# asalimil/Nonlinear-MPC-for-collision-free-and-deadlock-free-navigation-of-multiple-nonholonomic-mobile-robots

Hardware: AMD Instinct MI355X
Metric: NMPC solves/sec (batched swarms), N_robots=6, N=20 (higher is better)
Workload: dtype f64

## Files before the change

nonlinear-mpc-for-collision-free-and-deadlock-free-navigation-of-multiple-nonholonomic-mobile-robots_amd/csrc/nmpc_solve_col.hip:

```cpp
#include "nmpc_solve_common.h"

namespace nmpc {

__device__ __forceinline__ double lane_read(double v, int lane)
{
    return __hiloint2double(__builtin_amdgcn_readlane(__double2hiint(v), lane), __builtin_amdgcn_readlane(__double2loint(v), lane));
}
#ifndef NMPC_COL_GB
#define NMPC_COL_GB ((M_ == 6) ? (NX + 2) / 2 : NX + 1)
#endif
#ifndef NMPC_FW_PD
#define NMPC_FW_PD ((M_ <= 6) ? 2 : 1)
#endif
#ifndef NMPC_FW_FAKE
#define NMPC_FW_FAKE 0
#endif
#ifndef NMPC_COL_DPP
#define NMPC_COL_DPP 1
#endif
#ifndef NMPC_COL_WAVES_SMALL
#define NMPC_COL_WAVES_SMALL 1
#endif
#ifndef NMPC_COL_WAVES_MID
#define NMPC_COL_WAVES_MID 1
// ... 208 lines not shown
            for (int e = tid; e < N * NU; e += TPB) wo[(size_t)N1 * NX + e] = U[e];
            if (P.lam_g) for (int e = tid; e < P.ng; e += TPB) P.lam_g[inst * (size_t)P.ng + e] = 0.0;
            if (P.lam_x) for (int e = tid; e < P.nvar; e += TPB) P.lam_x[inst * (size_t)P.nvar + e] = 0.0;
            if (P.lam_p) for (int e = tid; e < 2 * NX; e += TPB) P.lam_p[inst * (size_t)(2 * NX) + e] = 0.0;
            if (tid == 0) {
                if (obj_out) obj_out[inst] = NAN;
                if (status_out) status_out[inst] = NMPC_STATUS_INFEASIBLE_X0;
                if (iters_out) iters_out[inst] = 0;
                if (kkt_out) kkt_out[inst] = INFINITY;
            }
            return;
        }
    }

    auto pair_ij = [&](int q, int &i, int &j) { pair_of<M_>(q, i, j); };

    auto trig = [&]() {
        for (int it = tid; it < N * M_; it += TPB) {
            int k = it / M_, i = it - k * M_;
            double s, c;
            sincos(X[k * NX + 3 * i + 2], &s, &c);
            SN[it] = s; CS[it] = c;
        }
    };
    auto merit_t = [&](auto elc, double a, double &fv, double &lg, double &th, double &ec_, double &eh_) {
        constexpr bool EL = decltype(elc)::value;
        double fs = 0.0, t = 0.0, mc = 0.0, mh = 0.0;
        LogSum ls;
        double pr = 1.0;
        auto brow = [&](double sv, double h0, double jd, double ht) {
            double st = sv + a * (jd + (h0 - sv));
            pr *= st;
            double r = fabs(ht - st);
            t += r; mh = fmax(mh, r);
        };
        for (int it = tid; it < N * M_; it += TPB) {
            int k = it / M_, i = it - k * M_;
            const int ox = k * NX + 3 * i, ou = k * NU + 2 * i;
            double x0 = X[ox] + a * DX[ox], x1 = X[ox + 1] + a * DX[ox + 1], x2 = X[ox + 2] + a * DX[ox + 2];
            double n0 = X[ox + NX] + a * DX[ox + NX], n1 = X[ox + NX + 1] + a * DX[ox + NX + 1], n2 = X[ox + NX + 2] + a * DX[ox + NX + 2];
            double u0 = U[ou] + a * DU[ou], u1 = U[ou + 1] + a * DU[ou + 1];
            double s, c;
            if (a == 0.0) { s = SN[it]; c = CS[it]; } else sincos(x2, &s, &c);
            double c0 = fabs(defect_xy(n0, x0, T * u0, c)), c1 = fabs(defect_xy(n1, x1, T * u0, s)), c2 = fabs(defect_th(n2, x2, T, u1));
            t += c0 + c1 + c2; mc = fmax(mc, fmax(c0, fmax(c1, c2)));
            double e0 = x0 - XS[3 * i], e1 = x1 - XS[3 * i + 1], e2 = x2 - XS[3 * i + 2];
            fs += P.q[0] * e0 * e0 + P.q[1] * e1 * e1 + P.q[2] * e2 * e2 + P.r[0] * u0 * u0 + P.r[1] * u1 * u1;
            brow(SUL[ou], U[ou] + P.vmax, DU[ou], u0 + P.vmax); brow(SUU[ou], P.vmax - U[ou], -DU[ou], P.vmax - u0);
            brow(SUL[ou + 1], U[ou + 1] + P.wmax, DU[ou + 1], u1 + P.wmax); brow(SUU[ou + 1], P.wmax - U[ou + 1], -DU[ou + 1], P.wmax - u1);
            pr *= ((n0 + P.xymax) * (P.xymax - n0)) * ((n1 + P.xymax) * (P.xymax - n1));
            if (THB) pr *= (n2 + P.thmax) * (P.thmax - n2);
            ls.add(pr);
            pr = 1.0;
        }
        for (int it = tid; it < (N - 1) * NPA; it += TPB) {
            int k = 1 + it / NPd, q = it - (k - 1) * NP, i, j;
            pair_ij(q, i, j);
            const int oi = k * NX + 3 * i, oj = k * NX + 3 * j;
            double dx = (X[oi] + a * DX[oi]) - (X[oj] + a * DX[oj]), dy = (X[oi + 1] + a * DX[oi + 1]) - (X[oj + 1] + a * DX[oj + 1]);
            double h = h_pair(dx, dy, P.dmin2);
            double sv = SPp[k * NP + q], tv = 0.0;
            if constexpr (EL) {
                tv = TPp[k * NP + q];
                if (a != 0.0) {
                    double ex = X[oi] - X[oj], ey = X[oi + 1] - X[oj + 1], ds, dz, dt;
                    el_step(mu, rho, sv, ZPp[k * NP + q], tv, h_pair(ex, ey, P.dmin2), jd_pair(ex, ey, DX[oi] - DX[oj], DX[oi + 1] - DX[oj + 1]), ds, dz, dt);
                    sv += a * ds; tv += a * dt;
                }
                ls.add(tv); fs += rho * tv;
            } else if (a != 0.0) {
                double ex = X[oi] - X[oj], ey = X[oi + 1] - X[oj + 1];
                sv += a * ds_pair(ex, ey, DX[oi] - DX[oj], DX[oi + 1] - DX[oj + 1], P.dmin2, sv);
            }
            ls.add(sv);
            double r = fabs(h - sv + tv);
            t += r; mh = fmax(mh, r);
        }
        for (int it = tid; it < (N - 1) * MK; it += TPB) {
            int k = 1 + it / MK, e = it - (k - 1) * MK, i = e / K, o = e - i * K;
            const int oi = k * NX + 3 * i;
            double px = X[oi] + a * DX[oi], py = X[oi + 1] + a * DX[oi + 1];
            double h = h_obs(r_obs(px - OB(k, o, 0), py - OB(k, o, 1)), P.robdim, OB(k, o, 2), P.margin);
            double sv = SO[k * MK + e], tv = 0.0;
            if constexpr (EL) {
                tv = TOb[k * MK + e];
                if (a != 0.0) {
                    double ex = X[oi] - OB(k, o, 0), ey = X[oi + 1] - OB(k, o, 1), rr = r_obs(ex, ey), ds, dz, dt;
                    el_step(mu, rho, sv, ZO[k * MK + e], tv, h_obs(rr, P.robdim, OB(k, o, 2), P.margin), jd_obs(ex, ey, rr, DX[oi], DX[oi + 1]), ds, dz, dt);
                    sv += a * ds; tv += a * dt;
                }
                ls.add(tv); fs += rho * tv;
            } else if (a != 0.0) {
                double ex = X[oi] - OB(k, o, 0), ey = X[oi + 1] - OB(k, o, 1), rr = r_obs(ex, ey);
// ... 3 lines not shown
            double r = fabs(h - sv + tv);
            t += r; mh = fmax(mh, r);
        }
        fv = wsum<TPB>(fs, RED); lg = wlogsum<TPB>(ls, RED); th = wsum<TPB>(t, RED);
        ec_ = wmax<TPB>(mc, RED); eh_ = wmax<TPB>(mh, RED);
    };
    auto merit = [&](double a, double &fv, double &lg, double &th, double &ec_, double &eh_) {
        if (el) merit_t(std::true_type{}, a, fv, lg, th, ec_, eh_); else merit_t(std::false_type{}, a, fv, lg, th, ec_, eh_);
    };

    for (int it = tid; it < N * M_; it += TPB) {
        int k = it / M_, i = it - k * M_;
        if (i == 0) { gpack[(size_t)k * G::PACK + G::PK_T] = T; gpack[(size_t)k * G::PACK + G::PK_ZERO] = 0.0; }
    }
    for (int q = tid; q < 3 * NP; q += TPB) gpack[G::PK_E + q] = 0.0;
    if (!prs)
        for (int e = tid; e < (N - 1) * 3 * NP; e += TPB) gpack[(size_t)(1 + e / (3 * NPd)) * G::PACK + G::PK_E + e % (3 * NPd)] = 0.0;
    auto init_barrier = [&]() {
        for (int it = tid; it < N1 * NP; it += TPB) {
            int k = it / NPd, q = it - k * NP;
            if (k >= 1 && k <= N - 1 && prs) {
                int i, j; pair_ij(q, i, j);
                double dx = X[k * NX + 3 * i] - X[k * NX + 3 * j], dy = X[k * NX + 3 * i + 1] - X[k * NX + 3 * j + 1];
                const double hv = h_pair(dx, dy, P.dmin2);
                if (el) {
                    const double tv = fmax(bp, bp - hv), sv = hv + tv;
                    TPp[it] = tv; SPp[it] = sv; ZPp[it] = fmin(mu / sv, 0.5 * rho);
                } else {
                double sv = fmax(hv, bp);
                SPp[it] = sv; ZPp[it] = mu / sv;
// ... 62 lines not shown
        }
        __syncthreads();
    }
    trig();
    __syncthreads();
    init_barrier();
    merit(0.0, f, lgs, th0, e_c, e_h);
    delta_last = 0.0; nu_pen = 1.0; need_shift = false; mcount = 0; restarting = false;
    PROF_T(0);

    for (;;) {
        double e_d = 0.0, lsum = 0.0, zsum = 0.0, szmax = 0.0, szmin = INFINITY;
#ifdef NMPC_PROFILE
        double dbg_code = -1.0, dbg_v[4] = {0, 0, 0, 0};
#endif
        for (int it = tid; it < N * M_; it += TPB) {
            int k = it / M_, i = it - k * M_, kk = k + 1;
            const double *x = X + kk * NX;
            double r0 = LAM[kk * NX + 3 * i], r1 = LAM[kk * NX + 3 * i + 1], r2 = LAM[kk * NX + 3 * i + 2];
            lsum += fabs(r0) + fabs(r1) + fabs(r2);
            if (kk < N) {
                const double *ln = LAM + (kk + 1) * NX + 3 * i;
                double v = U[kk * NU + 2 * i];
                double a = -T * v * SN[kk * M_ + i], b = T * v * CS[kk * M_ + i];
                r0 += 2 * P.q[0] * (x[3 * i] - XS[3 * i]) - ln[0];
                r1 += 2 * P.q[1] * (x[3 * i + 1] - XS[3 * i + 1]) - ln[1];
                r2 += 2 * P.q[2] * (x[3 * i + 2] - XS[3 * i + 2]) - (ln[2] + a * ln[0] + b * ln[1]);
            }
            double j0, j1, j2 = 0.0;
            {
                const int sb = kk * NXB + (2 + THB) * i;
                double zl0 = ZXL[sb], zu0 = ZXU[sb], zl1 = ZXL[sb + 1], zu1 = ZXU[sb + 1];
                j0 = zl0 - zu0; j1 = zl1 - zu1;
                zsum += zl0 + zu0 + zl1 + zu1;
                double p0 = (x[3 * i] + P.xymax) * zl0, p1 = (P.xymax - x[3 * i]) * zu0, p2 = (x[3 * i + 1] + P.xymax) * zl1, p3 = (P.xymax - x[3 * i + 1]) * zu1;
                szmax = fmax(szmax, fmax(fmax(p0, p1), fmax(p2, p3))); szmin = fmin(szmin, fmin(fmin(p0, p1), fmin(p2, p3)));
                if (THB) {
                    double zl2 = ZXL[sb + 2], zu2 = ZXU[sb + 2];
                    j2 = zl2 - zu2; zsum += zl2 + zu2;
                    double p4 = (x[3 * i + 2] + P.thmax) * zl2, p5 = (P.thmax - x[3 * i + 2]) * zu2;
                    szmax = fmax(szmax, fmax(p4, p5)); szmin = fmin(szmin, fmin(p4, p5));
                }
            }
            if (kk <= N - 1) {
                const double xi = x[3 * i], yi = x[3 * i + 1];
                if (prs) {
                    double zq[MPN];
                    static_for<0, M_ - 1>([&](auto pc) { constexpr int p = decltype(pc)::value; zq[p] = ZPp[kk * NP + pidx_any<M_>(i, p + (p >= i ? 1 : 0))]; });
                    static_for<0, M_ - 1>([&](auto pc) {
                        constexpr int p = decltype(pc)::value;
                        const int j = p + (p >= i ? 1 : 0);
                        j0 += 2 * (xi - x[3 * j]) * zq[p]; j1 += 2 * (yi - x[3 * j + 1]) * zq[p];
                    });
                }
                for (int o = 0; o < K; o++) {
                    double dx = xi - OB(kk, o, 0), dy = yi - OB(kk, o, 1), rr = r_obs(dx, dy), z = ZO[kk * MK + i * K + o];
                    j0 += qdiv(dx, rr) * z; j1 += qdiv(dy, rr) * z;
                }
            }
#ifdef NMPC_PROFILE
            { double m3 = fmax(fabs(r0 - j0), fmax(fabs(r1 - j1), fabs(r2 - j2)));
              if (m3 > e_d) { dbg_code = 1000.0 * kk + 10.0 * i + (fabs(r0 - j0) == m3 ? 0 : (fabs(r1 - j1) == m3 ? 1 : 2)); dbg_v[0] = r0 - j0; dbg_v[1] = r1 - j1; dbg_v[2] = r2 - j2; dbg_v[3] = r2; } }
#endif
            e_d = fmax(e_d, fmax(fabs(r0 - j0), fmax(fabs(r1 - j1), fabs(r2 - j2))));
            const double *ln = LAM + (k + 1) * NX + 3 * i, *u = U + k * NU + 2 * i;
            double c = CS[it], s = SN[it];
            double zl0 = ZUL[k * NU + 2 * i], zu0 = ZUU[k * NU + 2 * i], zl1 = ZUL[k * NU + 2 * i + 1], zu1 = ZUU[k * NU + 2 * i + 1];
            double rv = 2 * P.r[0] * u[0] - T * (c * ln[0] + s * ln[1]) - (zl0 - zu0);
            double rw = 2 * P.r[1] * u[1] - T * ln[2] - (zl1 - zu1);
#ifdef NMPC_PROFILE
            if (fmax(fabs(rv), fabs(rw)) > e_d) { dbg_code = 1000.0 * k + 10.0 * i + (fabs(rv) > fabs(rw) ? 5 : 6); dbg_v[0] = rv; dbg_v[1] = rw; dbg_v[2] = zl0 - zu0; dbg_v[3] = zl1 - zu1; }
#endif
            e_d = fmax(e_d, fmax(fabs(rv), fabs(rw)));
            zsum += zl0 + zu0 + zl1 + zu1;
            double p0 = SUL[k * NU + 2 * i] * zl0, p1 = SUU[k * NU + 2 * i] * zu0, p2 = SUL[k * NU + 2 * i + 1] * zl1, p3 = SUU[k * NU + 2 * i + 1] * zu1;
            szmax = fmax(szmax, fmax(fmax(p0, p1), fmax(p2, p3))); szmin = fmin(szmin, fmin(fmin(p0, p1), fmin(p2, p3)));
        }
        for (int it = tid; it < (N - 1) * NPA; it += TPB) {
            double zv = ZPp[NP + it], pz = SPp[NP + it] * zv;
            zsum += zv; szmax = fmax(szmax, pz); szmin = fmin(szmin, pz);
        }
        for (int it = tid; it < (N - 1) * MK; it += TPB) {
            double zv = ZO[MK + it], pz = SO[MK + it] * zv;
            zsum += zv; szmax = fmax(szmax, pz); szmin = fmin(szmin, pz);
        }
        if (el) {
            for (int it = tid; it < (N - 1) * NPA; it += TPB) { const double pt = TPp[NP + it] * (rho - ZPp[NP + it]); szmax = fmax(szmax, pt); szmin = fmin(szmin, pt); }
            for (int it = tid; it < (N - 1) * MK; it += TPB) { const double pt = TOb[MK + it] * (rho - ZO[MK + it]); szmax = fmax(szmax, pt); szmin = fmin(szmin, pt); }
        }
#ifdef NMPC_PROFILE
        { double my = e_d; double gm = wmax<TPB>(e_d, RED);
          if (prof_out && (int)inst == P.trace_inst && iter < 2040 && my == gm) {
              double *tr = reinterpret_cast<double *>(prof_out + 12 + 16 * 2048) + (size_t)iter * 8;
              tr[0] = dbg_code; tr[1] = dbg_v[0]; tr[2] = dbg_v[1]; tr[3] = dbg_v[2]; tr[4] = dbg_v[3]; } }
#endif
        e_d = wmax<TPB>(e_d, RED); lsum = wsum<TPB>(lsum, RED); zsum = wsum<TPB>(zsum, RED);
        szmax = wmax<TPB>(szmax, RED); szmin = wmin<TPB>(szmin, RED);
        const double smax = 100.0;
        double s_d = fmax(smax, (lsum + zsum) / ((double)(N * NX) + n_ineq)) / smax;
        double s_c = fmax(smax, zsum / fmax(n_ineq, 1.0)) / smax;
        double E0 = fmax(fmax(e_d / s_d, e_c), fmax(e_h, szmax / s_c));
        kkt = E0;
        auto cold_retry = [&]() { cold = true; n_cold++; it_base = iter; restarting = true; el = n_cold >= 2; mu = P.mu_init; n_tiny = 0; n_restart = 0; };
        if (!(E0 == E0)) { if (n_cold < NMPC_COLD_RETRIES && iter < P.max_iter) cold_retry(); else status = NMPC_STATUS_NUMERIC; break; }
        if (E0 <= P.tol) {
            status = NMPC_STATUS_CONVERGED;
            if (el) {
                double tmax = 0.0;
                for (int it = tid; it < (N - 1) * NPA; it += TPB) tmax = fmax(tmax, TPp[NP + it]);
                for (int it = tid; it < (N - 1) * MK; it += TPB) tmax = fmax(tmax, TOb[MK + it]);
                if (wmax<TPB>(tmax, RED) > NMPC_X0_TOL) status = NMPC_STATUS_STALLED;
            }
            break;
        }
        if (iter >= P.max_iter) { status = NMPC_STATUS_MAX_ITER; break; }
        if (n_cold < NMPC_COLD_RETRIES && iter - it_base >= NMPC_COLD_RETRY_ITERS) { cold_retry(); break; }
        const double mu_min = P.tol / 10.0;
        for (;;) {
            double cm = fmax(fabs(szmax - mu), fabs(szmin - mu));
            double Emu = fmax(fmax(e_d / s_d, e_c), fmax(e_h, cm / s_c));
            if (mu > mu_min && Emu <= 10.0 * mu) mu = fmax(mu_min, fmin(0.2 * mu, pow(mu, 1.5)));
            else break;
        }
        const double tau = fmax(0.99, 1.0 - mu);
        PROF_T(1);

        auto stage_packs = [&](auto elc) {
        constexpr bool EL = decltype(elc)::value;
        for (int it = tid; it < N1 * M_; it += TPB) {
            int k = it / M_, i = it - k * M_;
            const double *x = X + k * NX;
            double *pk = gpack + (size_t)k * G::PACK;
            double g0 = 0.0, g1 = 0.0, g2 = 0.0, h0 = 0.0, h1 = 0.0, h2 = 0.0, hxy = 0.0;
            if (k >= 1) {
                if (k < N) {
                    g0 = 2 * P.q[0] * (x[3 * i] - XS[3 * i]); g1 = 2 * P.q[1] * (x[3 * i + 1] - XS[3 * i + 1]); g2 = 2 * P.q[2] * (x[3 * i + 2] - XS[3 * i + 2]);
                    h0 = 2 * P.q[0]; h1 = 2 * P.q[1]; h2 = 2 * P.q[2];
                }
                const int sb = k * NXB + (2 + THB) * i;
                {
                    auto bv = [&](double sv, double zv, double hv, double &hd) { double sg = qdiv(zv, sv); hd += sg; return qdiv(mu, sv) - sg * (hv - sv); };
                    g0 -= bv(x[3 * i] + P.xymax, ZXL[sb], x[3 * i] + P.xymax, h0) - bv(P.xymax - x[3 * i], ZXU[sb], P.xymax - x[3 * i], h0);
                    g1 -= bv(x[3 * i + 1] + P.xymax, ZXL[sb + 1], x[3 * i + 1] + P.xymax, h1) - bv(P.xymax - x[3 * i + 1], ZXU[sb + 1], P.xymax - x[3 * i + 1], h1);
                    if (THB) g2 -= bv(x[3 * i + 2] + P.thmax, ZXL[sb + 2], x[3 * i + 2] + P.thmax, h2) - bv(P.thmax - x[3 * i + 2], ZXU[sb + 2], P.thmax - x[3 * i + 2], h2);
// ... 44 lines not shown
                }
                {
                    double *cf = pk + G::PK_CF + 4 * i;
                    cf[0] = T * c; cf[1] = T * s; cf[2] = -T * u[0] * s; cf[3] = T * u[0] * c;
                }
                const double *xn = x + NX;
                pk[G::PK_C + 3 * i] = defect_xy(xn[3 * i], x[3 * i], T * u[0], c);
                pk[G::PK_C + 3 * i + 1] = defect_xy(xn[3 * i + 1], x[3 * i + 1], T * u[0], s);
                pk[G::PK_C + 3 * i + 2] = defect_th(xn[3 * i + 2], x[3 * i + 2], T, u[1]);
                pk[G::PK_HVT + i] = hvt;
            }
            pk[G::PK_G + NU + 3 * i] = g0; pk[G::PK_G + NU + 3 * i + 1] = g1; pk[G::PK_G + NU + 3 * i + 2] = g2;
            pk[G::PK_HD + NU + 3 * i] = h0; pk[G::PK_HD + NU + 3 * i + 1] = h1; pk[G::PK_HD + NU + 3 * i + 2] = h2;
            pk[G::PK_HXY + i] = hxy;
        }
        for (int it = tid; it < (N - 1) * NPA; it += TPB) {
            int k = 1 + it / NPd, q = it - (k - 1) * NP, i, j;
            pair_ij(q, i, j);
            double dx = X[k * NX + 3 * i] - X[k * NX + 3 * j], dy = X[k * NX + 3 * i + 1] - X[k * NX + 3 * j + 1];
            double zz = ZPp[k * NP + q], sg;
            if constexpr (EL) { double v_; el_sigma(mu, rho, SPp[k * NP + q], zz, TPp[k * NP + q], h_pair(dx, dy, P.dmin2), sg, v_); }
            else sg = qdiv(zz, SPp[k * NP + q]);
            double *pk = gpack + (size_t)k * G::PACK + G::PK_E + 3 * q;
            pk[0] = -(4 * sg * dx * dx - 2 * zz); pk[1] = -(4 * sg * dx * dy); pk[2] = -(4 * sg * dy * dy - 2 * zz);
        }
        };
        if (el) stage_packs(std::true_type{}); else stage_packs(std::false_type{});
        __syncthreads();
        PROF_T(2);

        double delta = need_shift ? fmax(1e-20, 0.25 * delta_last) : 0.0;
        int ntry = 0;
        bool ok;
        int kst = N - 1;
        for (;;) {
            ok = true;
            int kf = 0;
            if (TPBK == 64 || tid < 64) {
            constexpr int TPB = 64;
            if constexpr (RP) {
            const int rh = tid >> 5, rw = (tid >> 4) & 1, rn = tid & 15;
            const bool cc_ = rn < NC;
// ... 477 lines not shown
#if NMPC_FUSE_DPHI
            dphi_b += qdiv(ds, sv);
#endif
            return zv + dz;
        };
        auto fbe = [&](double sv, double zv, double tv, double hv, double jd) -> double {
            double ds, dz, dt;
            el_step(mu, rho, sv, zv, tv, hv, jd, ds, dz, dt);
            if (ds < 0.0) a_p = fmin(a_p, qdiv(-tau * sv, ds));
            if (dt < 0.0) a_p = fmin(a_p, qdiv(-tau * tv, dt));
            if (dz < 0.0) a_d = fmin(a_d, qdiv(-tau * zv, dz));
            if (dz > 0.0) a_d = fmin(a_d, qdiv(tau * (rho - zv), dz));
            dphi_b += qdiv(ds, sv) + qdiv(dt, tv) - qdiv(rho, mu) * dt;
            return zv + dz;
        };
        for (int e = tid; e < N * NU; e += TPB) {
            int c = e % NU;
            double lo = lbu(c), u = U[e], du = DU[e], sl = SUL[e], su = SUU[e];
            fb(sl, ZUL[e], du + ((u - lo) - sl)); fb(su, ZUU[e], -du + ((-lo - u) - su));
        }
        for (int e = tid; e < N * NXB; e += TPB) {
            int k = 1 + e / NXB, s = e - (k - 1) * NXB;
            double v = X[k * NX + bst(s)], dv = DX[k * NX + bst(s)], b = bvl(s), sl = v + b, su = b - v;
            fb(sl, ZXL[k * NXB + s], dv + ((v + b) - sl)); fb(su, ZXU[k * NXB + s], -dv + ((b - v) - su));
        }
        if (!el) {
        for (int it = tid; it < (N - 1) * NPA; it += TPB) {
            int k = 1 + it / NPd, q = it - (k - 1) * NP, i, j;
            pair_ij(q, i, j);
            const int oi = k * NX + 3 * i, oj = k * NX + 3 * j;
            double ex = X[oi] - X[oj], ey = X[oi + 1] - X[oj + 1], sv = SPp[k * NP + q];
            double ds = ds_pair(ex, ey, DX[oi] - DX[oj], DX[oi + 1] - DX[oj + 1], P.dmin2, sv);
            mult_max = fmax(mult_max, fabs(fb(sv, ZPp[k * NP + q], ds)));
        }
        for (int it = tid; it < (N - 1) * MK; it += TPB) {
            int k = 1 + it / MK, e = it - (k - 1) * MK, i = e / K, o = e - i * K;
            const int oi = k * NX + 3 * i;
            double ex = X[oi] - OB(k, o, 0), ey = X[oi + 1] - OB(k, o, 1), rr = r_obs(ex, ey), sv = SO[k * MK + e];
            double ds = ds_obs(ex, ey, rr, DX[oi], DX[oi + 1], h_obs(rr, P.robdim, OB(k, o, 2), P.margin), sv);
            mult_max = fmax(mult_max, fabs(fb(sv, ZO[k * MK + e], ds)));
        }
        } else {
        for (int it = tid; it < (N - 1) * NPA; it += TPB) {
            int k = 1 + it / NPd, q = it - (k - 1) * NP, i, j;
            pair_ij(q, i, j);
            const int oi = k * NX + 3 * i, oj = k * NX + 3 * j;
            double ex = X[oi] - X[oj], ey = X[oi + 1] - X[oj + 1];
            mult_max = fmax(mult_max, fabs(fbe(SPp[k * NP + q], ZPp[k * NP + q], TPp[k * NP + q], h_pair(ex, ey, P.dmin2), jd_pair(ex, ey, DX[oi] - DX[oj], DX[oi + 1] - DX[oj + 1]))));
        }
        for (int it = tid; it < (N - 1) * MK; it += TPB) {
            int k = 1 + it / MK, e = it - (k - 1) * MK, i = e / K, o = e - i * K;
            const int oi = k * NX + 3 * i;
            double ex = X[oi] - OB(k, o, 0), ey = X[oi + 1] - OB(k, o, 1), rr = r_obs(ex, ey);
            mult_max = fmax(mult_max, fabs(fbe(SO[k * MK + e], ZO[k * MK + e], TOb[k * MK + e], h_obs(rr, P.robdim, OB(k, o, 2), P.margin), jd_obs(ex, ey, rr, DX[oi], DX[oi + 1]))));
        }
        }
        a_p = wmin<TPB>(a_p, RED); a_d = wmin<TPB>(a_d, RED);
        PROF_T(5);
        auto multiplier_residuals = [&](auto elc) {
        constexpr bool EL = decltype(elc)::value;
        for (int it = tid; it < N * M_; it += TPB) {
            int k = 1 + it / M_, i = it - (k - 1) * M_;
            const double *x = X + k * NX, *dx = DX + k * NX;
            double l0, l1, l2 = 0.0;
            {
                const int sb = k * NXB + (2 + THB) * i;
                auto zn = [&](double sv, double zv, double hv, double jd) { double ds = jd + (hv - sv); return zv + dz_of(mu, sv, zv, ds); };
                l0 = zn(x[3 * i] + P.xymax, ZXL[sb], x[3 * i] + P.xymax, dx[3 * i]) - zn(P.xymax - x[3 * i], ZXU[sb], P.xymax - x[3 * i], -dx[3 * i]);
                l1 = zn(x[3 * i + 1] + P.xymax, ZXL[sb + 1], x[3 * i + 1] + P.xymax, dx[3 * i + 1]) - zn(P.xymax - x[3 * i + 1], ZXU[sb + 1], P.xymax - x[3 * i + 1], -dx[3 * i + 1]);
                if (THB) l2 = zn(x[3 * i + 2] + P.thmax, ZXL[sb + 2], x[3 * i + 2] + P.thmax, dx[3 * i + 2]) - zn(P.thmax - x[3 * i + 2], ZXU[sb + 2], P.thmax - x[3 * i + 2], -dx[3 * i + 2]);
            }
            if (k < N) {
                const double xi = x[3 * i], yi = x[3 * i + 1];
                if (prs) {
                    double sq[MPN], zq[MPN];
                    static_for<0, M_ - 1>([&](auto pc) {
// ... 57 lines not shown
                    double a = -T * v * SN[k * M_ + i], b = T * v * CS[k * M_ + i];
                    l0 += n0; l1 += n1; l2 += n2 + a * n0 + b * n1;
                }
                n0 = l0; n1 = l1; n2 = l2;
                RV[k * NX + 3 * i] = l0; RV[k * NX + 3 * i + 1] = l1; RV[k * NX + 3 * i + 2] = l2;
                mult_max = fmax(mult_max, fmax(fabs(l0), fmax(fabs(l1), fabs(l2))));
            }
        }
        mult_max = wmax<TPB>(mult_max, RED);
        __syncthreads();
        PROF_T(7);


        double dphi = 0.0;
#if NMPC_FUSE_DPHI
        for (int it = tid; it < N * M_; it += TPB) {
            int k = it / M_, i = it - k * M_;
            if (k >= 1) {
#pragma unroll
                for (int d = 0; d < 3; d++) dphi += 2 * P.q[d] * (X[k * NX + 3 * i + d] - XS[3 * i + d]) * DX[k * NX + 3 * i + d];
            }
#pragma unroll
            for (int d = 0; d < 2; d++) { const int eu = k * NU + 2 * i + d; dphi += 2 * P.r[d] * U[eu] * DU[eu]; }
        }
        dphi -= mu * dphi_b;
#else
        for (int it = tid; it < N1 * M_; it += TPB) {
            int k = it / M_, i = it - k * M_;
            if (k >= 1 && k < N) {
#pragma unroll
                for (int d = 0; d < 3; d++) dphi += 2 * P.q[d] * (X[k * NX + 3 * i + d] - XS[3 * i + d]) * DX[k * NX + 3 * i + d];
            }
            if (k < N) {
#pragma unroll
                for (int d = 0; d < 2; d++) {
                    const int eu = k * NU + 2 * i + d;
                    double u = U[eu], du = DU[eu], lo = d ? -P.wmax : -P.vmax, sl = SUL[eu], su = SUU[eu];
                    dphi += 2 * P.r[d] * u * du - mu * ((du + ((u - lo) - sl)) / sl + (-du + ((-lo - u) - su)) / su);
                }
            }
            if (k >= 1) {
#pragma unroll
                for (int d = 0; d < 2 + THB; d++) {
                    const int sb = k * NXB + (2 + THB) * i + d;
                    double v = X[k * NX + 3 * i + d], dv = DX[k * NX + 3 * i + d], b = (d == 2) ? P.thmax : P.xymax, sl = v + b, su = b - v;
                    dphi -= mu * ((dv + ((v + b) - sl)) / sl + (-dv + ((b - v) - su)) / su);
                }
            }
        }
#endif
#if !NMPC_FUSE_DPHI
        for (int it = tid; it < (N - 1) * NPA; it += TPB) {
            int k = 1 + it / NPd, q = it - (k - 1) * NP, i, j;
            pair_ij(q, i, j);
            const int oi = k * NX + 3 * i, oj = k * NX + 3 * j;
            double ex = X[oi] - X[oj], ey = X[oi + 1] - X[oj + 1], sv = SPp[k * NP + q];
            double ds = ds_pair(ex, ey, DX[oi] - DX[oj], DX[oi + 1] - DX[oj + 1], P.dmin2, sv);
            dphi -= mu * ds / sv;
        }
        for (int it = tid; it < (N - 1) * MK; it += TPB) {
            int k = 1 + it / MK, e = it - (k - 1) * MK, i = e / K, o = e - i * K;
            const int oi = k * NX + 3 * i;
            double ex = X[oi] - OB(k, o, 0), ey = X[oi + 1] - OB(k, o, 1), rr = r_obs(ex, ey), sv = SO[k * MK + e];
            double ds = ds_obs(ex, ey, rr, DX[oi], DX[oi + 1], h_obs(rr, P.robdim, OB(k, o, 2), P.margin), sv);
            dphi -= mu * ds / sv;
        }
#endif
        dphi = wsum<TPB>(dphi, RED);
        const double phi0 = f - mu * lgs;
        if (th0 > 0.0) {
            double nut = fmin(dphi / ((1.0 - 0.1) * th0), mult_max / (1.0 - 0.1));
            nu_pen = fmax(1.0, 0.5 * nu_pen);
            if (nu_pen < nut) nu_pen = nut + 1.0;
        }
        const double Dm = dphi - nu_pen * th0;
// ... 30 lines not shown
#endif

        auto zup = [&](double sv, double zv, double ds, double &snew) {
            double dz = dz_of(mu, sv, zv, ds);
            snew = sv + alpha * ds;
            double z = zv + a_d * dz;
            return fmin(fmax(z, qdiv(1e-10 * mu, snew)), qdiv(1e10 * mu, snew));
        };
        auto zupe = [&](double sv, double zv, double tv, double hv, double jd, double &snew, double &tnew) {
            double ds, dz, dt;
            el_step(mu, rho, sv, zv, tv, hv, jd, ds, dz, dt);
            snew = sv + alpha * ds; tnew = tv + alpha * dt;
            double z = zv + a_d * dz;
            return fmin(fmax(z, qdiv(1e-10 * mu, snew)), fmin(qdiv(1e10 * mu, snew), rho - qdiv(1e-10 * mu, tnew)));
        };
        for (int e = tid; e < N * NU; e += TPB) {
            int c = e % NU;
            double lo = lbu(c), u = U[e], du = DU[e], sl = SUL[e], su = SUU[e], sn;
            ZUL[e] = zup(sl, ZUL[e], du + ((u - lo) - sl), sn); SUL[e] = sn;
            ZUU[e] = zup(su, ZUU[e], -du + ((-lo - u) - su), sn); SUU[e] = sn;
        }
        for (int e = tid; e < N * NXB; e += TPB) {
            int k = 1 + e / NXB, s = e - (k - 1) * NXB;
            const int es = k * NXB + s;
            double v = X[k * NX + bst(s)], dv = DX[k * NX + bst(s)], b = bvl(s), sl = v + b, su = b - v, sn;
            ZXL[es] = zup(sl, ZXL[es], dv + ((v + b) - sl), sn);
            ZXU[es] = zup(su, ZXU[es], -dv + ((b - v) - su), sn);
        }
        if (!el) {
        for (int it = tid; it < (N - 1) * NPA; it += TPB) {
            int k = 1 + it / NPd, q = it - (k - 1) * NP, i, j;
            pair_ij(q, i, j);
            const int oi = k * NX + 3 * i, oj = k * NX + 3 * j;
            double ex = X[oi] - X[oj], ey = X[oi + 1] - X[oj + 1], sv = SPp[k * NP + q], sn;
            double ds = ds_pair(ex, ey, DX[oi] - DX[oj], DX[oi + 1] - DX[oj + 1], P.dmin2, sv);
            ZPp[k * NP + q] = zup(sv, ZPp[k * NP + q], ds, sn);
            SPp[k * NP + q] = sn;
        }
        for (int it = tid; it < (N - 1) * MK; it += TPB) {
            int k = 1 + it / MK, e = it - (k - 1) * MK, i = e / K, o = e - i * K;
            const int oi = k * NX + 3 * i;
            double ex = X[oi] - OB(k, o, 0), ey = X[oi + 1] - OB(k, o, 1), rr = r_obs(ex, ey), sv = SO[k * MK + e], sn;
            double ds = ds_obs(ex, ey, rr, DX[oi], DX[oi + 1], h_obs(rr, P.robdim, OB(k, o, 2), P.margin), sv);
            ZO[k * MK + e] = zup(sv, ZO[k * MK + e], ds, sn);
            SO[k * MK + e] = sn;
        }
        } else {
        for (int it = tid; it < (N - 1) * NPA; it += TPB) {
            int k = 1 + it / NPd, q = it - (k - 1) * NP, i, j;
            pair_ij(q, i, j);
            const int oi = k * NX + 3 * i, oj = k * NX + 3 * j;
            double ex = X[oi] - X[oj], ey = X[oi + 1] - X[oj + 1], sn, tn;
            ZPp[k * NP + q] = zupe(SPp[k * NP + q], ZPp[k * NP + q], TPp[k * NP + q], h_pair(ex, ey, P.dmin2), jd_pair(ex, ey, DX[oi] - DX[oj], DX[oi + 1] - DX[oj + 1]), sn, tn);
            SPp[k * NP + q] = sn; TPp[k * NP + q] = tn;
        }
        for (int it = tid; it < (N - 1) * MK; it += TPB) {
            int k = 1 + it / MK, e = it - (k - 1) * MK, i = e / K, o = e - i * K;
            const int oi = k * NX + 3 * i;
            double ex = X[oi] - OB(k, o, 0), ey = X[oi + 1] - OB(k, o, 1), rr = r_obs(ex, ey), sn, tn;
            ZO[k * MK + e] = zupe(SO[k * MK + e], ZO[k * MK + e], TOb[k * MK + e], h_obs(rr, P.robdim, OB(k, o, 2), P.margin), jd_obs(ex, ey, rr, DX[oi], DX[oi + 1]), sn, tn);
            SO[k * MK + e] = sn; TOb[k * MK + e] = tn;
        }
        }
        __syncthreads();
        for (int e = tid; e < N1 * NX; e += TPB) { X[e] += alpha * DX[e]; if (e >= NX) LAM[e] += alpha * (RV[e] - LAM[e]); }
        for (int e = tid; e < N * NU; e += TPB) U[e] += alpha * DU[e];
        __syncthreads();
        trig();
        __syncthreads();
        f = ft; lgs = lgt; th0 = tht; e_c = ect; e_h = eht;
        iter++;
        PROF_T(8);
        if (n_tiny >= 5) {
            if (n_restart >= 3) { if (n_cold < NMPC_COLD_RETRIES) cold_retry(); else status = NMPC_STATUS_STALLED; break; }
            n_restart++; n_tiny = 0;
            mu = fmax(mu, P.mu_init);
            restarting = true;
            break;
        }
    }
    if (!restarting) break;
// ... 187 lines not shown
```

Baseline: 278,700.

## Fuse stage Hessian/gradient pack construction into optimality-error pass when mu unchanged

When there are no obstacles and no elastic mode, the optimality-error loop now also computes and writes the per-stage gradient, Hessian diagonal, dynamics coefficients, defects and pair packs. The later stage_packs pass is skipped unless mu changes after the error check, in which case only the stage part is recomputed. This saves a second sweep over states and multipliers per iteration. It also adds an asm barrier on tid to stop the compiler hoisting or rematerialising loop indices, at the cost of extra register pressure in the fused loop.

```diff
diff --git a/nonlinear-mpc-for-collision-free-and-deadlock-free-navigation-of-multiple-nonholonomic-mobile-robots_amd/csrc/nmpc_solve_col.hip b/nonlinear-mpc-for-collision-free-and-deadlock-free-navigation-of-multiple-nonholonomic-mobile-robots_amd/csrc/nmpc_solve_col.hip
--- a/nonlinear-mpc-for-collision-free-and-deadlock-free-navigation-of-multiple-nonholonomic-mobile-robots_amd/csrc/nmpc_solve_col.hip
+++ b/nonlinear-mpc-for-collision-free-and-deadlock-free-navigation-of-multiple-nonholonomic-mobile-robots_amd/csrc/nmpc_solve_col.hip
@@ -246,6 +246,7 @@
     }
 
     auto pair_ij = [&](int q, int &i, int &j) { pair_of<M_>(q, i, j); };
+    auto tid_local = [&]() { int t = tid; asm volatile("" : "+v"(t)); return t; };
 
     auto trig = [&]() {
         for (int it = tid; it < N * M_; it += TPB) {
@@ -266,7 +267,7 @@
             double r = fabs(ht - st);
             t += r; mh = fmax(mh, r);
         };
-        for (int it = tid; it < N * M_; it += TPB) {
+        for (int it = tid_local(); it < N * M_; it += TPB) {
             int k = it / M_, i = it - k * M_;
             const int ox = k * NX + 3 * i, ou = k * NU + 2 * i;
             double x0 = X[ox] + a * DX[ox], x1 = X[ox + 1] + a * DX[ox + 1], x2 = X[ox + 2] + a * DX[ox + 2];
@@ -285,7 +286,7 @@
             ls.add(pr);
             pr = 1.0;
         }
-        for (int it = tid; it < (N - 1) * NPA; it += TPB) {
+        for (int it = tid_local(); it < (N - 1) * NPA; it += TPB) {
             int k = 1 + it / NPd, q = it - (k - 1) * NP, i, j;
             pair_ij(q, i, j);
             const int oi = k * NX + 3 * i, oj = k * NX + 3 * j;
@@ -308,7 +309,7 @@
             double r = fabs(h - sv + tv);
             t += r; mh = fmax(mh, r);
         }
-        for (int it = tid; it < (N - 1) * MK; it += TPB) {
+        for (int it = tid_local(); it < (N - 1) * MK; it += TPB) {
             int k = 1 + it / MK, e = it - (k - 1) * MK, i = e / K, o = e - i * K;
             const int oi = k * NX + 3 * i;
             double px = X[oi] + a * DX[oi], py = X[oi + 1] + a * DX[oi + 1];
@@ -342,6 +343,11 @@
         if (i == 0) { gpack[(size_t)k * G::PACK + G::PK_T] = T; gpack[(size_t)k * G::PACK + G::PK_ZERO] = 0.0; }
     }
     for (int q = tid; q < 3 * NP; q += TPB) gpack[G::PK_E + q] = 0.0;
+    for (int i = tid; i < M_; i += TPB) {
+#pragma unroll
+        for (int d = 0; d < 3; d++) { gpack[G::PK_G + NU + 3 * i + d] = 0.0; gpack[G::PK_HD + NU + 3 * i + d] = 0.0; }
+        gpack[G::PK_HXY + i] = 0.0;
+    }
     if (!prs)
         for (int e = tid; e < (N - 1) * 3 * NP; e += TPB) gpack[(size_t)(1 + e / (3 * NPd)) * G::PACK + G::PK_E + e % (3 * NPd)] = 0.0;
     auto init_barrier = [&]() {
@@ -434,18 +440,28 @@
 #ifdef NMPC_PROFILE
         double dbg_code = -1.0, dbg_v[4] = {0, 0, 0, 0};
 #endif
-        for (int it = tid; it < N * M_; it += TPB) {
+        auto opt_err = [&](auto fzc) {
+        constexpr bool FZ = decltype(fzc)::value;
+        for (int it = tid_local(); it < N * M_; it += TPB) {
             int k = it / M_, i = it - k * M_, kk = k + 1;
             const double *x = X + kk * NX;
             double r0 = LAM[kk * NX + 3 * i], r1 = LAM[kk * NX + 3 * i + 1], r2 = LAM[kk * NX + 3 * i + 2];
             lsum += fabs(r0) + fabs(r1) + fabs(r2);
+            double g0 = 0.0, g1 = 0.0, g2 = 0.0, h0 = 0.0, h1 = 0.0, h2 = 0.0, hxy = 0.0;
+            double vn = 0.0, sk = 0.0, ck = 0.0, ln0 = 0.0, ln1 = 0.0;
             if (kk < N) {
                 const double *ln = LAM + (kk + 1) * NX + 3 * i;
                 double v = U[kk * NU + 2 * i];
-                double a = -T * v * SN[kk * M_ + i], b = T * v * CS[kk * M_ + i];
+                sk = SN[kk * M_ + i]; ck = CS[kk * M_ + i];
+                double a = -T * v * sk, b = T * v * ck;
                 r0 += 2 * P.q[0] * (x[3 * i] - XS[3 * i]) - ln[0];
                 r1 += 2 * P.q[1] * (x[3 * i + 1] - XS[3 * i + 1]) - ln[1];
                 r2 += 2 * P.q[2] * (x[3 * i + 2] - XS[3 * i + 2]) - (ln[2] + a * ln[0] + b * ln[1]);
+                if constexpr (FZ) {
+                    g0 = 2 * P.q[0] * (x[3 * i] - XS[3 * i]); g1 = 2 * P.q[1] * (x[3 * i + 1] - XS[3 * i + 1]); g2 = 2 * P.q[2] * (x[3 * i + 2] - XS[3 * i + 2]);
+                    h0 = 2 * P.q[0]; h1 = 2 * P.q[1]; h2 = 2 * P.q[2];
+                    vn = v; ln0 = ln[0]; ln1 = ln[1];
+                }
             }
             double j0, j1, j2 = 0.0;
             {
@@ -455,22 +471,41 @@
                 zsum += zl0 + zu0 + zl1 + zu1;
                 double p0 = (x[3 * i] + P.xymax) * zl0, p1 = (P.xymax - x[3 * i]) * zu0, p2 = (x[3 * i + 1] + P.xymax) * zl1, p3 = (P.xymax - x[3 * i + 1]) * zu1;
                 szmax = fmax(szmax, fmax(fmax(p0, p1), fmax(p2, p3))); szmin = fmin(szmin, fmin(fmin(p0, p1), fmin(p2, p3)));
+                double zl2 = 0.0, zu2 = 0.0;
                 if (THB) {
-                    double zl2 = ZXL[sb + 2], zu2 = ZXU[sb + 2];
+                    zl2 = ZXL[sb + 2]; zu2 = ZXU[sb + 2];
                     j2 = zl2 - zu2; zsum += zl2 + zu2;
                     double p4 = (x[3 * i + 2] + P.thmax) * zl2, p5 = (P.thmax - x[3 * i + 2]) * zu2;
                     szmax = fmax(szmax, fmax(p4, p5)); szmin = fmin(szmin, fmin(p4, p5));
                 }
+                if constexpr (FZ) {
+                    auto bv = [&](double sv, double zv, double hv, double &hd) { double sg = qdiv(zv, sv); hd += sg; return qdiv(mu, sv) - sg * (hv - sv); };
+                    g0 -= bv(x[3 * i] + P.xymax, zl0, x[3 * i] + P.xymax, h0) - bv(P.xymax - x[3 * i], zu0, P.xymax - x[3 * i], h0);
+                    g1 -= bv(x[3 * i + 1] + P.xymax, zl1, x[3 * i + 1] + P.xymax, h1) - bv(P.xymax - x[3 * i + 1], zu1, P.xymax - x[3 * i + 1], h1);
+                    if (THB) g2 -= bv(x[3 * i + 2] + P.thmax, zl2, x[3 * i + 2] + P.thmax, h2) - bv(P.thmax - x[3 * i + 2], zu2, P.thmax - x[3 * i + 2], h2);
+                }
             }
             if (kk <= N - 1) {
                 const double xi = x[3 * i], yi = x[3 * i + 1];
                 if (prs) {
-                    double zq[MPN];
-                    static_for<0, M_ - 1>([&](auto pc) { constexpr int p = decltype(pc)::value; zq[p] = ZPp[kk * NP + pidx_any<M_>(i, p + (p >= i ? 1 : 0))]; });
+                    double zq[MPN], sq[MPN];
+                    static_for<0, M_ - 1>([&](auto pc) {
+                        constexpr int p = decltype(pc)::value;
+                        const int q = pidx_any<M_>(i, p + (p >= i ? 1 : 0));
+                        zq[p] = ZPp[kk * NP + q];
+                        if constexpr (FZ) sq[p] = SPp[kk * NP + q];
+                    });
                     static_for<0, M_ - 1>([&](auto pc) {
                         constexpr int p = decltype(pc)::value;
                         const int j = p + (p >= i ? 1 : 0);
                         j0 += 2 * (xi - x[3 * j]) * zq[p]; j1 += 2 * (yi - x[3 * j + 1]) * zq[p];
+                        if constexpr (FZ) {
+                            double dx = xi - x[3 * j], dy = yi - x[3 * j + 1];
+                            double sv = sq[p], zv = zq[p], sg, v;
+                            sg = qdiv(zv, sv); v = qdiv(mu, sv) - sg * (h_pair(dx, dy, P.dmin2) - sv);
+                            g0 -= 2 * dx * v; g1 -= 2 * dy * v;
+                            h0 += 4 * sg * dx * dx - 2 * zv; hxy += 4 * sg * dx * dy; h1 += 4 * sg * dy * dy - 2 * zv;
+                        }
                     });
                 }
                 for (int o = 0; o < K; o++) {
@@ -478,6 +513,7 @@
                     j0 += qdiv(dx, rr) * z; j1 += qdiv(dy, rr) * z;
                 }
             }
+            if constexpr (FZ) { if (kk < N) h2 += T * vn * (ln0 * ck + ln1 * sk); }
 #ifdef NMPC_PROFILE
             { double m3 = fmax(fabs(r0 - j0), fmax(fabs(r1 - j1), fabs(r2 - j2)));
               if (m3 > e_d) { dbg_code = 1000.0 * kk + 10.0 * i + (fabs(r0 - j0) == m3 ? 0 : (fabs(r1 - j1) == m3 ? 1 : 2)); dbg_v[0] = r0 - j0; dbg_v[1] = r1 - j1; dbg_v[2] = r2 - j2; dbg_v[3] = r2; } }
@@ -485,6 +521,7 @@
             e_d = fmax(e_d, fmax(fabs(r0 - j0), fmax(fabs(r1 - j1), fabs(r2 - j2))));
             const double *ln = LAM + (k + 1) * NX + 3 * i, *u = U + k * NU + 2 * i;
             double c = CS[it], s = SN[it];
+            const double sl0 = SUL[k * NU + 2 * i], su0 = SUU[k * NU + 2 * i], sl1 = SUL[k * NU + 2 * i + 1], su1 = SUU[k * NU + 2 * i + 1];
             double zl0 = ZUL[k * NU + 2 * i], zu0 = ZUU[k * NU + 2 * i], zl1 = ZUL[k * NU + 2 * i + 1], zu1 = ZUU[k * NU + 2 * i + 1];
             double rv = 2 * P.r[0] * u[0] - T * (c * ln[0] + s * ln[1]) - (zl0 - zu0);
             double rw = 2 * P.r[1] * u[1] - T * ln[2] - (zl1 - zu1);
@@ -493,20 +530,57 @@
 #endif
             e_d = fmax(e_d, fmax(fabs(rv), fabs(rw)));
             zsum += zl0 + zu0 + zl1 + zu1;
-            double p0 = SUL[k * NU + 2 * i] * zl0, p1 = SUU[k * NU + 2 * i] * zu0, p2 = SUL[k * NU + 2 * i + 1] * zl1, p3 = SUU[k * NU + 2 * i + 1] * zu1;
+            double p0 = sl0 * zl0, p1 = su0 * zu0, p2 = sl1 * zl1, p3 = su1 * zu1;
             szmax = fmax(szmax, fmax(fmax(p0, p1), fmax(p2, p3))); szmin = fmin(szmin, fmin(fmin(p0, p1), fmin(p2, p3)));
-        }
-        for (int it = tid; it < (N - 1) * NPA; it += TPB) {
-            double zv = ZPp[NP + it], pz = SPp[NP + it] * zv;
+            if constexpr (FZ) {
+                const double *xk = X + k * NX;
+                double *pk = gpack + (size_t)k * G::PACK, *pn = gpack + (size_t)kk * G::PACK;
+                const double hvt = T * (ln[0] * s - ln[1] * c);
+                double pg[2], ph[2];
+#pragma unroll
+                for (int d = 0; d < 2; d++) {
+                    double lo = d ? -P.wmax : -P.vmax, sl = d ? sl1 : sl0, su = d ? su1 : su0, zl = d ? zl1 : zl0, zu = d ? zu1 : zu0;
+                    double vl = qdiv(mu, sl) - qdiv(zl, sl) * ((u[d] - lo) - sl), vu = qdiv(mu, su) - qdiv(zu, su) * ((-lo - u[d]) - su);
+                    pg[d] = 2 * P.r[d] * u[d] - (vl - vu);
+                    ph[d] = 2 * P.r[d] + qdiv(zl, sl) + qdiv(zu, su);
+                }
+                const double d0 = defect_xy(x[3 * i], xk[3 * i], T * u[0], c), d1 = defect_xy(x[3 * i + 1], xk[3 * i + 1], T * u[0], s), d2 = defect_th(x[3 * i + 2], xk[3 * i + 2], T, u[1]);
+                const double cf0 = T * c, cf1_ = T * s, cf2 = -T * u[0] * s, cf3 = T * u[0] * c;
+                pk[G::PK_G + 2 * i] = pg[0]; pk[G::PK_G + 2 * i + 1] = pg[1];
+                pk[G::PK_HD + 2 * i] = ph[0]; pk[G::PK_HD + 2 * i + 1] = ph[1];
+                {
+                    double *cf = pk + G::PK_CF + 4 * i;
+                    cf[0] = cf0; cf[1] = cf1_; cf[2] = cf2; cf[3] = cf3;
+                }
+                pk[G::PK_C + 3 * i] = d0; pk[G::PK_C + 3 * i + 1] = d1; pk[G::PK_C + 3 * i + 2] = d2;
+                pk[G::PK_HVT + i] = hvt;
+                pn[G::PK_G + NU + 3 * i] = g0; pn[G::PK_G + NU + 3 * i + 1] = g1; pn[G::PK_G + NU + 3 * i + 2] = g2;
+                pn[G::PK_HD + NU + 3 * i] = h0; pn[G::PK_HD + NU + 3 * i + 1] = h1; pn[G::PK_HD + NU + 3 * i + 2] = h2;
+                pn[G::PK_HXY + i] = hxy;
+            }
+        }
+        for (int it = tid_local(); it < (N - 1) * NPA; it += TPB) {
+            double zv = ZPp[NP + it], sv = SPp[NP + it], pz = sv * zv;
             zsum += zv; szmax = fmax(szmax, pz); szmin = fmin(szmin, pz);
-        }
-        for (int it = tid; it < (N - 1) * MK; it += TPB) {
+            if constexpr (FZ) {
+                int k = 1 + it / NPd, q = it - (k - 1) * NP, i, j;
+                pair_ij(q, i, j);
+                double dx = X[k * NX + 3 * i] - X[k * NX + 3 * j], dy = X[k * NX + 3 * i + 1] - X[k * NX + 3 * j + 1];
+                double zz = zv, sg = qdiv(zz, sv);
+                double *pk = gpack + (size_t)k * G::PACK + G::PK_E + 3 * q;
+                pk[0] = -(4 * sg * dx * dx - 2 * zz); pk[1] = -(4 * sg * dx * dy); pk[2] = -(4 * sg * dy * dy - 2 * zz);
+            }
+        }
+        };
+        const bool fuse_packs = !el && K == 0;
+        if (fuse_packs) opt_err(std::true_type{}); else opt_err(std::false_type{});
+        for (int it = tid_local(); it < (N - 1) * MK; it += TPB) {
             double zv = ZO[MK + it], pz = SO[MK + it] * zv;
             zsum += zv; szmax = fmax(szmax, pz); szmin = fmin(szmin, pz);
         }
         if (el) {
-            for (int it = tid; it < (N - 1) * NPA; it += TPB) { const double pt = TPp[NP + it] * (rho - ZPp[NP + it]); szmax = fmax(szmax, pt); szmin = fmin(szmin, pt); }
-            for (int it = tid; it < (N - 1) * MK; it += TPB) { const double pt = TOb[MK + it] * (rho - ZO[MK + it]); szmax = fmax(szmax, pt); szmin = fmin(szmin, pt); }
+            for (int it = tid_local(); it < (N - 1) * NPA; it += TPB) { const double pt = TPp[NP + it] * (rho - ZPp[NP + it]); szmax = fmax(szmax, pt); szmin = fmin(szmin, pt); }
+            for (int it = tid_local(); it < (N - 1) * MK; it += TPB) { const double pt = TOb[MK + it] * (rho - ZO[MK + it]); szmax = fmax(szmax, pt); szmin = fmin(szmin, pt); }
         }
 #ifdef NMPC_PROFILE
         { double my = e_d; double gm = wmax<TPB>(e_d, RED);
@@ -527,8 +601,8 @@
             status = NMPC_STATUS_CONVERGED;
             if (el) {
                 double tmax = 0.0;
-                for (int it = tid; it < (N - 1) * NPA; it += TPB) tmax = fmax(tmax, TPp[NP + it]);
-                for (int it = tid; it < (N - 1) * MK; it += TPB) tmax = fmax(tmax, TOb[MK + it]);
+                for (int it = tid_local(); it < (N - 1) * NPA; it += TPB) tmax = fmax(tmax, TPp[NP + it]);
+                for (int it = tid_local(); it < (N - 1) * MK; it += TPB) tmax = fmax(tmax, TOb[MK + it]);
                 if (wmax<TPB>(tmax, RED) > NMPC_X0_TOL) status = NMPC_STATUS_STALLED;
             }
             break;
@@ -536,6 +610,7 @@
         if (iter >= P.max_iter) { status = NMPC_STATUS_MAX_ITER; break; }
         if (n_cold < NMPC_COLD_RETRIES && iter - it_base >= NMPC_COLD_RETRY_ITERS) { cold_retry(); break; }
         const double mu_min = P.tol / 10.0;
+        const double mu_packs = mu;
         for (;;) {
             double cm = fmax(fabs(szmax - mu), fabs(szmin - mu));
             double Emu = fmax(fmax(e_d / s_d, e_c), fmax(e_h, cm / s_c));
@@ -545,9 +620,9 @@
         const double tau = fmax(0.99, 1.0 - mu);
         PROF_T(1);
 
-        auto stage_packs = [&](auto elc) {
+        auto stage_packs_a = [&](auto elc) {
         constexpr bool EL = decltype(elc)::value;
-        for (int it = tid; it < N1 * M_; it += TPB) {
+        for (int it = tid_local(); it < N1 * M_; it += TPB) {
             int k = it / M_, i = it - k * M_;
             const double *x = X + k * NX;
             double *pk = gpack + (size_t)k * G::PACK;
@@ -622,7 +697,10 @@
             pk[G::PK_HD + NU + 3 * i] = h0; pk[G::PK_HD + NU + 3 * i + 1] = h1; pk[G::PK_HD + NU + 3 * i + 2] = h2;
             pk[G::PK_HXY + i] = hxy;
         }
-        for (int it = tid; it < (N - 1) * NPA; it += TPB) {
+        };
+        auto stage_packs_b = [&](auto elc) {
+        constexpr bool EL = decltype(elc)::value;
+        for (int it = tid_local(); it < (N - 1) * NPA; it += TPB) {
             int k = 1 + it / NPd, q = it - (k - 1) * NP, i, j;
             pair_ij(q, i, j);
             double dx = X[k * NX + 3 * i] - X[k * NX + 3 * j], dy = X[k * NX + 3 * i + 1] - X[k * NX + 3 * j + 1];
@@ -633,7 +711,9 @@
             pk[0] = -(4 * sg * dx * dx - 2 * zz); pk[1] = -(4 * sg * dx * dy); pk[2] = -(4 * sg * dy * dy - 2 * zz);
         }
         };
-        if (el) stage_packs(std::true_type{}); else stage_packs(std::false_type{});
+        if (el) { stage_packs_a(std::true_type{}); stage_packs_b(std::true_type{}); }
+        else if (!fuse_packs) { stage_packs_a(std::false_type{}); stage_packs_b(std::false_type{}); }
+        else if (mu != mu_packs) stage_packs_a(std::false_type{});
         __syncthreads();
         PROF_T(2);
 
@@ -1141,18 +1221,18 @@
             dphi_b += qdiv(ds, sv) + qdiv(dt, tv) - qdiv(rho, mu) * dt;
             return zv + dz;
         };
-        for (int e = tid; e < N * NU; e += TPB) {
+        for (int e = tid_local(); e < N * NU; e += TPB) {
             int c = e % NU;
             double lo = lbu(c), u = U[e], du = DU[e], sl = SUL[e], su = SUU[e];
             fb(sl, ZUL[e], du + ((u - lo) - sl)); fb(su, ZUU[e], -du + ((-lo - u) - su));
         }
-        for (int e = tid; e < N * NXB; e += TPB) {
+        for (int e = tid_local(); e < N * NXB; e += TPB) {
             int k = 1 + e / NXB, s = e - (k - 1) * NXB;
             double v = X[k * NX + bst(s)], dv = DX[k * NX + bst(s)], b = bvl(s), sl = v + b, su = b - v;
             fb(sl, ZXL[k * NXB + s], dv + ((v + b) - sl)); fb(su, ZXU[k * NXB + s], -dv + ((b - v) - su));
         }
         if (!el) {
-        for (int it = tid; it < (N - 1) * NPA; it += TPB) {
+        for (int it = tid_local(); it < (N - 1) * NPA; it += TPB) {
             int k = 1 + it / NPd, q = it - (k - 1) * NP, i, j;
             pair_ij(q, i, j);
             const int oi = k * NX + 3 * i, oj = k * NX + 3 * j;
@@ -1160,7 +1240,7 @@
             double ds = ds_pair(ex, ey, DX[oi] - DX[oj], DX[oi + 1] - DX[oj + 1], P.dmin2, sv);
             mult_max = fmax(mult_max, fabs(fb(sv, ZPp[k * NP + q], ds)));
         }
-        for (int it = tid; it < (N - 1) * MK; it += TPB) {
+        for (int it = tid_local(); it < (N - 1) * MK; it += TPB) {
             int k = 1 + it / MK, e = it - (k - 1) * MK, i = e / K, o = e - i * K;
             const int oi = k * NX + 3 * i;
             double ex = X[oi] - OB(k, o, 0), ey = X[oi + 1] - OB(k, o, 1), rr = r_obs(ex, ey), sv = SO[k * MK + e];
@@ -1168,14 +1248,14 @@
             mult_max = fmax(mult_max, fabs(fb(sv, ZO[k * MK + e], ds)));
         }
         } else {
-        for (int it = tid; it < (N - 1) * NPA; it += TPB) {
+        for (int it = tid_local(); it < (N - 1) * NPA; it += TPB) {
             int k = 1 + it / NPd, q = it - (k - 1) * NP, i, j;
             pair_ij(q, i, j);
             const int oi = k * NX + 3 * i, oj = k * NX + 3 * j;
             double ex = X[oi] - X[oj], ey = X[oi + 1] - X[oj + 1];
             mult_max = fmax(mult_max, fabs(fbe(SPp[k * NP + q], ZPp[k * NP + q], TPp[k * NP + q], h_pair(ex, ey, P.dmin2), jd_pair(ex, ey, DX[oi] - DX[oj], DX[oi + 1] - DX[oj + 1]))));
         }
-        for (int it = tid; it < (N - 1) * MK; it += TPB) {
+        for (int it = tid_local(); it < (N - 1) * MK; it += TPB) {
             int k = 1 + it / MK, e = it - (k - 1) * MK, i = e / K, o = e - i * K;
             const int oi = k * NX + 3 * i;
             double ex = X[oi] - OB(k, o, 0), ey = X[oi + 1] - OB(k, o, 1), rr = r_obs(ex, ey);
@@ -1186,7 +1266,7 @@
         PROF_T(5);
         auto multiplier_residuals = [&](auto elc) {
         constexpr bool EL = decltype(elc)::value;
-        for (int it = tid; it < N * M_; it += TPB) {
+        for (int it = tid_local(); it < N * M_; it += TPB) {
             int k = 1 + it / M_, i = it - (k - 1) * M_;
             const double *x = X + k * NX, *dx = DX + k * NX;
             double l0, l1, l2 = 0.0;
@@ -1274,7 +1354,7 @@
 
         double dphi = 0.0;
 #if NMPC_FUSE_DPHI
-        for (int it = tid; it < N * M_; it += TPB) {
+        for (int it = tid_local(); it < N * M_; it += TPB) {
             int k = it / M_, i = it - k * M_;
             if (k >= 1) {
 #pragma unroll
@@ -1285,7 +1365,7 @@
         }
         dphi -= mu * dphi_b;
 #else
-        for (int it = tid; it < N1 * M_; it += TPB) {
+        for (int it = tid_local(); it < N1 * M_; it += TPB) {
             int k = it / M_, i = it - k * M_;
             if (k >= 1 && k < N) {
 #pragma unroll
@@ -1310,7 +1390,7 @@
         }
 #endif
 #if !NMPC_FUSE_DPHI
-        for (int it = tid; it < (N - 1) * NPA; it += TPB) {
+        for (int it = tid_local(); it < (N - 1) * NPA; it += TPB) {
             int k = 1 + it / NPd, q = it - (k - 1) * NP, i, j;
             pair_ij(q, i, j);
             const int oi = k * NX + 3 * i, oj = k * NX + 3 * j;
@@ -1318,7 +1398,7 @@
             double ds = ds_pair(ex, ey, DX[oi] - DX[oj], DX[oi + 1] - DX[oj + 1], P.dmin2, sv);
             dphi -= mu * ds / sv;
         }
-        for (int it = tid; it < (N - 1) * MK; it += TPB) {
+        for (int it = tid_local(); it < (N - 1) * MK; it += TPB) {
             int k = 1 + it / MK, e = it - (k - 1) * MK, i = e / K, o = e - i * K;
             const int oi = k * NX + 3 * i;
             double ex = X[oi] - OB(k, o, 0), ey = X[oi + 1] - OB(k, o, 1), rr = r_obs(ex, ey), sv = SO[k * MK + e];
@@ -1379,13 +1459,13 @@
             double z = zv + a_d * dz;
             return fmin(fmax(z, qdiv(1e-10 * mu, snew)), fmin(qdiv(1e10 * mu, snew), rho - qdiv(1e-10 * mu, tnew)));
         };
-        for (int e = tid; e < N * NU; e += TPB) {
+        for (int e = tid_local(); e < N * NU; e += TPB) {
             int c = e % NU;
             double lo = lbu(c), u = U[e], du = DU[e], sl = SUL[e], su = SUU[e], sn;
             ZUL[e] = zup(sl, ZUL[e], du + ((u - lo) - sl), sn); SUL[e] = sn;
             ZUU[e] = zup(su, ZUU[e], -du + ((-lo - u) - su), sn); SUU[e] = sn;
         }
-        for (int e = tid; e < N * NXB; e += TPB) {
+        for (int e = tid_local(); e < N * NXB; e += TPB) {
             int k = 1 + e / NXB, s = e - (k - 1) * NXB;
             const int es = k * NXB + s;
             double v = X[k * NX + bst(s)], dv = DX[k * NX + bst(s)], b = bvl(s), sl = v + b, su = b - v, sn;
@@ -1393,7 +1473,7 @@
             ZXU[es] = zup(su, ZXU[es], -dv + ((b - v) - su), sn);
         }
         if (!el) {
-        for (int it = tid; it < (N - 1) * NPA; it += TPB) {
+        for (int it = tid_local(); it < (N - 1) * NPA; it += TPB) {
             int k = 1 + it / NPd, q = it - (k - 1) * NP, i, j;
             pair_ij(q, i, j);
             const int oi = k * NX + 3 * i, oj = k * NX + 3 * j;
@@ -1402,7 +1482,7 @@
             ZPp[k * NP + q] = zup(sv, ZPp[k * NP + q], ds, sn);
             SPp[k * NP + q] = sn;
         }
-        for (int it = tid; it < (N - 1) * MK; it += TPB) {
+        for (int it = tid_local(); it < (N - 1) * MK; it += TPB) {
             int k = 1 + it / MK, e = it - (k - 1) * MK, i = e / K, o = e - i * K;
             const int oi = k * NX + 3 * i;
             double ex = X[oi] - OB(k, o, 0), ey = X[oi + 1] - OB(k, o, 1), rr = r_obs(ex, ey), sv = SO[k * MK + e], sn;
@@ -1411,7 +1491,7 @@
             SO[k * MK + e] = sn;
         }
         } else {
-        for (int it = tid; it < (N - 1) * NPA; it += TPB) {
+        for (int it = tid_local(); it < (N - 1) * NPA; it += TPB) {
             int k = 1 + it / NPd, q = it - (k - 1) * NP, i, j;
             pair_ij(q, i, j);
             const int oi = k * NX + 3 * i, oj = k * NX + 3 * j;
@@ -1419,7 +1499,7 @@
             ZPp[k * NP + q] = zupe(SPp[k * NP + q], ZPp[k * NP + q], TPp[k * NP + q], h_pair(ex, ey, P.dmin2), jd_pair(ex, ey, DX[oi] - DX[oj], DX[oi + 1] - DX[oj + 1]), sn, tn);
             SPp[k * NP + q] = sn; TPp[k * NP + q] = tn;
         }
-        for (int it = tid; it < (N - 1) * MK; it += TPB) {
+        for (int it = tid_local(); it < (N - 1) * MK; it += TPB) {
             int k = 1 + it / MK, e = it - (k - 1) * MK, i = e / K, o = e - i * K;
             const int oi = k * NX + 3 * i;
             double ex = X[oi] - OB(k, o, 0), ey = X[oi + 1] - OB(k, o, 1), rr = r_obs(ex, ey), sn, tn;
@@ -1428,8 +1508,8 @@
         }
         }
         __syncthreads();
-        for (int e = tid; e < N1 * NX; e += TPB) { X[e] += alpha * DX[e]; if (e >= NX) LAM[e] += alpha * (RV[e] - LAM[e]); }
-        for (int e = tid; e < N * NU; e += TPB) U[e] += alpha * DU[e];
+        for (int e = tid_local(); e < N1 * NX; e += TPB) { X[e] += alpha * DX[e]; if (e >= NX) LAM[e] += alpha * (RV[e] - LAM[e]); }
+        for (int e = tid_local(); e < N * NU; e += TPB) U[e] += alpha * DU[e];
         __syncthreads();
         trig();
         __syncthreads();
```

New measurement: 283,100 (median of 6 runs). 1.02x the previous value.
